# vismaychuriwala/Fast-Image-Editing-with-Generative-Models

Measured on AMD Instinct MI355X. Metric: PIE-Bench images/sec @1024^2 SSD-1B fp16 4-step, higher is better.
Workload: dtype f16

## Files before the change

fast-image-editing-with-generative-models_amd/csrc/fie_internal.h:

```cpp
#pragma once
#include <hip/hip_runtime.h>
#include <stdint.h>
#include <stdio.h>
#include <string.h>
#include <map>
#include <string>
#include <tuple>
#include <utility>
#include <vector>
#include "../../include/fie.h"

typedef _Float16 half_t;
typedef _Float16 f16x8 __attribute__((ext_vector_type(8)));
typedef _Float16 f16x4 __attribute__((ext_vector_type(4)));
typedef _Float16 f16x2 __attribute__((ext_vector_type(2)));
typedef float f32x4 __attribute__((ext_vector_type(4)));
typedef short s16x4 __attribute__((ext_vector_type(4)));
typedef unsigned u32x4 __attribute__((ext_vector_type(4)));

struct fie_launch_rec {
    const void* fn;
    dim3 grid, block;
    unsigned lds;
    std::vector<unsigned char> blob;
// ... 19 lines not shown
};

struct fie_ctx {
    int device;
    hipStream_t stream;
    int num_cus;
    int force_tile = 0;
    int gemm_probe = 0;
    int epi_prefetch = 1;
    unsigned* gemm_stamps = nullptr;
    float* gn_target = nullptr;
    int64_t gn_target_rows = 0;
    int gn_target_groups = 0;
    int attn_variant = 0;
    int gn_onepass = 1;
    unsigned* err_flag = nullptr;
    void* sk_ws = nullptr;
    int64_t sk_bytes = 0;
    int splitk_mode = 1;
    int autotune = 0;
    std::map<fie_tune_key, int> tuned;
    int tune_exclude[16] = {0};
    void* tune_buf = nullptr;
    void* tune_flush = nullptr;
    size_t tune_bytes = 0;
    int n_overrides = 0;
    fie_tile_override overrides[32];
    char last_kernel[128] = "";
    fie_program* recording = nullptr;
    std::vector<std::string>* oplog = nullptr;
// ... 94 lines not shown
```

fast-image-editing-with-generative-models_amd/csrc/graphs.cpp:

```cpp
#include <string>
#include <vector>

#include "fie_internal.h"

namespace {

struct Arena {
    struct Blk { int64_t off, size; bool used; };
    std::vector<Blk> blks;
    int64_t high = 0;
    explicit Arena(int64_t cap) { blks.push_back({0, cap, false}); }
    int64_t take(int64_t bytes) {
        bytes = fie_roundup(bytes > 0 ? bytes : 1, 256);
        for (size_t i = 0; i < blks.size(); ++i) {
            if (blks[i].used || blks[i].size < bytes) continue;
            const int64_t off = blks[i].off, rest = blks[i].size - bytes;
            blks[i].size = bytes;
            blks[i].used = true;
            if (rest > 0) blks.insert(blks.begin() + i + 1, Blk{off + bytes, rest, false});
            if (off + bytes > high) high = off + bytes;
            return off;
        }
        return -1;
    }
// ... 27 lines not shown
    int rc = FIE_OK;
    bool plan_fused = true;
    char* cache = nullptr;
    int64_t cache_cap = 0, cache_cur = 0;
    bool cache_fill = false, cache_count = false;
    bool cached() const { return cache != nullptr || cache_count; }
    T cache_slot(int64_t rows, int c) {
        T t;
        t.rows = rows; t.c = c;
        const int64_t bytes = fie_roundup(rows * c * 2, 256);
        if (!cache_count && cache_cur + bytes > cache_cap && rc == FIE_OK) { fie_set_error("%s: step cache too small (fie_unet_step_cache_bytes)", who); rc = FIE_EINVAL; }
        t.ext = cache_count || !ok() ? reinterpret_cast<void*>(1) : static_cast<void*>(cache + cache_cur);
        cache_cur += bytes;
        return t;
    }
    Walk(fie_ctx* c, const char* w, const char* pre, void* ws, int64_t cap) : ctx(c), who(w), prefix(pre ? pre : ""), base(static_cast<char*>(ws)), arena(cap) {}
    bool plan() const { return ctx == nullptr; }
    bool ok() const { return rc == FIE_OK; }
    void run(int r) { if (rc == FIE_OK && r != FIE_OK) rc = r; }

    T alloc(int64_t rows, int c) {
        T t;
        t.rows = rows; t.c = c;
        t.off = arena.take(rows * c * 2);
        if (t.off < 0 && rc == FIE_OK) { fie_set_error("%s: workspace too small", who); rc = FIE_EINVAL; t.off = 0; }
        return t;
    }
    int64_t scratch(int64_t bytes) {
        int64_t off = arena.take(bytes);
        if (off < 0 && rc == FIE_OK) { fie_set_error("%s: workspace too small", who); rc = FIE_EINVAL; off = 0; }
        return off;
// ... 685 lines not shown
```

fast-image-editing-with-generative-models_amd/csrc/norm.hip:

```cpp
#include "fie_internal.h"

namespace {

constexpr int GN_THREADS = 256;
constexpr int GN_MAX_CHUNKS = 1024;

template <typename T>
struct GnArgsT {
    const T* X1; int C1;
    const T* X2; int C2;
    T* Y;
    int C, G, cg;
    int64_t rows;
    int rows_per_chunk, nchunks;
    int ncol;
    int rpp;
    const T* gamma; const T* beta;
    float eps; int silu;
    float* partial;
    float* stats;
    float o8_inv;
    int pg;
};

using GnArgs = GnArgsT<half_t>;

__device__ __forceinline__ int gn_pack4_f8(const float* o, float inv) {
    auto q = [&](float x) { return fie_sat448(x * inv); };
    int pk = __builtin_amdgcn_cvt_pk_fp8_f32(q(o[0]), q(o[1]), 0, false);
    return __builtin_amdgcn_cvt_pk_fp8_f32(q(o[2]), q(o[3]), pk, true);
}

template <typename T>
__device__ __forceinline__ void gn_load(const GnArgsT<T>& p, int64_t row_global, int c0, float (&x)[8]) {
    if (c0 < p.C1) fie_load8(p.X1 + row_global * p.C1 + c0, x);
    else fie_load8(p.X2 + row_global * p.C2 + (c0 - p.C1), x);
}

template <typename T>
__global__ __launch_bounds__(GN_THREADS) void gn_partial_kernel(GnArgsT<T> p) {
    __shared__ float red[GN_THREADS * 16];
    const int tid = threadIdx.x;
    const int col = tid % p.ncol, rsub = tid / p.ncol;
    const int b = blockIdx.y;
    const int c0 = (blockIdx.z * p.ncol + col) * 8;
    const bool active = rsub < p.rpp && c0 < p.C;
    float s[8], ss[8];
#pragma unroll
    for (int j = 0; j < 8; ++j) s[j] = ss[j] = 0.f;
    if (active) {
        const int64_t r_begin = (int64_t)blockIdx.x * p.rows_per_chunk;
// ... 16 lines not shown
    __syncthreads();
    const int cbase = blockIdx.z * p.ncol * 8;
    const int cend = min(cbase + p.ncol * 8, p.C);
    const int g_first = cbase / p.cg, g_last = (cend - 1) / p.cg;
    for (int g = g_first + tid; g <= g_last; g += GN_THREADS) {
        float a = 0.f, q = 0.f;
        const int ch_lo = max(g * p.cg, cbase), ch_hi = min((g + 1) * p.cg, cend);
        for (int ch = ch_lo; ch < ch_hi; ++ch) {
            const int lc = (ch - cbase) >> 3, j = (ch - cbase) & 7;
            for (int rs = 0; rs < p.rpp; ++rs) {
                a += red[(rs * p.ncol + lc) * 16 + j];
                q += red[(rs * p.ncol + lc) * 16 + 8 + j];
            }
        }
        float* dst = p.partial + (((int64_t)b * p.nchunks + blockIdx.x) * p.G + g) * 2;
        dst[0] = a;
        dst[1] = q;
    }
}

template <typename T>
__global__ __launch_bounds__(256) void gn_finalize_kernel(GnArgsT<T> p, int B) {
    const int lane = threadIdx.x & 63;
    const int i = blockIdx.x * 4 + (threadIdx.x >> 6);
    if (i >= B * p.G) return;
    const int b = i / p.G, g = i - b * p.G;
    double a = 0.0, q = 0.0;
    for (int c = lane; c < p.nchunks; c += 64) {
        const float2 v = *reinterpret_cast<const float2*>(p.partial + (((int64_t)b * p.nchunks + c) * p.G + g) * 2);
        a += (double)v.x;
        q += (double)v.y;
    }
#pragma unroll
    for (int o = 32; o > 0; o >>= 1) {
        a += __shfl_xor(a, o);
        q += __shfl_xor(q, o);
    }
    if (lane == 0) {
        const double n = (double)p.rows * p.cg;
        const double mean = a / n;
        double var = q / n - mean * mean;
        if (var < 0.0) var = 0.0;
        p.stats[i * 2] = (float)mean;
        p.stats[i * 2 + 1] = (float)(1.0 / sqrt(var + (double)p.eps));
    }
}

template <typename T>
__global__ __launch_bounds__(256) void gn_finalize_wide_kernel(GnArgsT<T> p, int B) {
    __shared__ double red[8];
    const int tid = threadIdx.x, lane = tid & 63, wave = tid >> 6;
    const int i = blockIdx.x;
    const int b = i / p.G, g = i - b * p.G;
    double a0 = 0.0, q0 = 0.0, a1 = 0.0, q1 = 0.0, a2 = 0.0, q2 = 0.0, a3 = 0.0, q3 = 0.0;
    if (p.pg > p.G) {
        const int upg = p.pg / p.G;
        const float2* src = reinterpret_cast<const float2*>(p.partial) + (int64_t)b * p.nchunks * p.pg + g * upg;
        const int total = p.nchunks * upg;
        for (int i = tid; i < total; i += 256) {
            const int c = i / upg, u = i - c * upg;
// ... 39 lines not shown
    const int tid = threadIdx.x, g = tid % p.G, sub = tid / p.G, nsub = 256 / p.G;
    const int b = blockIdx.y, c0 = blockIdx.x * per, c1 = min(c0 + per, ngran);
    const float2* src = reinterpret_cast<const float2*>(granules) + (int64_t)b * ngran * p.G + g;
    double a0 = 0.0, q0 = 0.0, a1 = 0.0, q1 = 0.0;
    int c = c0 + sub;
    for (; c + nsub < c1; c += 2 * nsub) {
        const float2 v0 = src[(int64_t)c * p.G], v1 = src[(int64_t)(c + nsub) * p.G];
        a0 += (double)v0.x; q0 += (double)v0.y; a1 += (double)v1.x; q1 += (double)v1.y;
    }
    if (c < c1) { const float2 v = src[(int64_t)c * p.G]; a0 += (double)v.x; q0 += (double)v.y; }
    red[tid][0] = a0 + a1; red[tid][1] = q0 + q1;
    __syncthreads();
    if (sub == 0) {
        double a = 0.0, q = 0.0;
        for (int s = 0; s < nsub; ++s) { a += red[s * p.G + g][0]; q += red[s * p.G + g][1]; }
        *reinterpret_cast<float2*>(p.partial + (((int64_t)b * gridDim.x + blockIdx.x) * p.G + g) * 2) = make_float2((float)a, (float)q);
    }
}

template <typename T>
__global__ __launch_bounds__(GN_THREADS) void gn_apply_kernel(GnArgsT<T> p) {
    const int tid = threadIdx.x;
    const int col = tid % p.ncol, rsub = tid / p.ncol;
    const int b = blockIdx.y;
    const int c0 = (blockIdx.z * p.ncol + col) * 8;
    if (!(rsub < p.rpp && c0 < p.C)) return;
    float sc[8], sh[8];
    float gm[8], bt[8];
    fie_load8(p.gamma + c0, gm);
    fie_load8(p.beta + c0, bt);
#pragma unroll
    for (int j = 0; j < 8; ++j) {
// ... 239 lines not shown
                fie_store8(Y + row * ldy + ch * 8, o);
            }
        }
    }
}

template <typename T, bool O8, typename... Args>
void ln_launch(fie_ctx* ctx, int64_t rows, int C, Args... args) {
    const dim3 grid((unsigned)((rows + 3) / 4)), block(256);
    if (C <= 1024) fie_launch(ctx, (ln_kernel<T, O8, 2>), grid, block, 0, args...);
    else if (C <= 1536) fie_launch(ctx, (ln_kernel<T, O8, 3>), grid, block, 0, args...);
    else fie_launch(ctx, (ln_kernel<T, O8, LN_MAXV>), grid, block, 0, args...);
}

template <typename T>
int gn_plan(GnArgsT<T>& p, int C, int G, int64_t rows, int B, int* csplit) {
    const int nc8 = C / 8;
    int split = (nc8 + GN_THREADS - 1) / GN_THREADS;
    while (split <= nc8 && (nc8 % split != 0 || ((nc8 / split) * 8) % (C / G) != 0)) ++split;
    if (split > nc8) return -1;
    p.ncol = nc8 / split;
    p.rpp = GN_THREADS / p.ncol;
    *csplit = split;
    int64_t want = 2048 / (B > 0 ? B : 1);
    if (want < 1) want = 1;
    if (want > GN_MAX_CHUNKS) want = GN_MAX_CHUNKS;
    int64_t rpc = fie_roundup((rows + want - 1) / want, p.rpp);
    int64_t nch = (rows + rpc - 1) / rpc;
    p.rows_per_chunk = (int)rpc;
    p.nchunks = (int)nch;
    return 0;
}

template <typename T>
int groupnorm_t(const char* who, fie_ctx* ctx, const void* X1, int C1, const void* X2, int C2, void* Y, int B, int64_t rows_per_image,
                int groups, const void* gamma, const void* beta, float eps, int silu, void* workspace, float o8_inv = 0.f) {
    FIE_REQUIRE(ctx && X1 && Y && gamma && beta && workspace, "%s: NULL argument", who);
    FIE_REQUIRE(C1 > 0 && C1 % 8 == 0 && C2 >= 0 && C2 % 8 == 0 && (C2 == 0 || X2), "%s: C1=%d C2=%d invalid", who, C1, C2);
    const int C = C1 + C2;
    FIE_REQUIRE(B > 0 && rows_per_image > 0 && groups > 0 && C % groups == 0, "%s: bad shape C=%d G=%d", who, C, groups);
    GnArgsT<T> p = {};
    p.X1 = (const T*)X1; p.C1 = C1; p.X2 = (const T*)X2; p.C2 = C2; p.Y = (T*)Y;
    p.C = C; p.G = groups; p.cg = C / groups; p.rows = rows_per_image;
    p.gamma = (const T*)gamma; p.beta = (const T*)beta; p.eps = eps; p.silu = silu;
    p.o8_inv = o8_inv;
    int csplit = 1;
    FIE_REQUIRE(gn_plan(p, C, groups, rows_per_image, B, &csplit) == 0, "%s: cannot split C=%d (groups=%d) into aligned column blocks", who, C, groups);
    if (ctx->gn_onepass && gn_onepass(ctx, p, B)) {
        FIE_LAUNCH_CHECK();
        return FIE_OK;
    }
    p.partial = (float*)workspace;
    p.stats = p.partial + (int64_t)B * GN_MAX_CHUNKS * groups * 2;
    const dim3 grid((unsigned)p.nchunks, (unsigned)B, (unsigned)csplit);
    FIE_DESC(ctx, "groupnorm partial B=%d rows=%lld C=%d G=%d bytes=%.0f", B, (long long)rows_per_image, C, groups, 1.0 * B * rows_per_image * C * sizeof(T));
    fie_launch(ctx, gn_partial_kernel<T>, grid, dim3(GN_THREADS), 0, p);
    FIE_DESC(ctx, "groupnorm finalize B=%d rows=%lld C=%d G=%d bytes=0", B, (long long)rows_per_image, C, groups);
    fie_launch(ctx, gn_finalize_kernel<T>, dim3((B * groups + 3) / 4), dim3(256), 0, p, B);
    FIE_DESC(ctx, "groupnorm apply B=%d rows=%lld C=%d G=%d bytes=%.0f", B, (long long)rows_per_image, C, groups, 2.0 * B * rows_per_image * C * sizeof(T));
    fie_launch(ctx, gn_apply_kernel<T>, grid, dim3(GN_THREADS), 0, p);
    FIE_LAUNCH_CHECK();
    return FIE_OK;
}

template <typename T>
int layernorm_t(const char* who, fie_ctx* ctx, const void* X, int64_t ldx, void* Y, int64_t ldy, int64_t rows, int C, const void* gamma,
                const void* beta, float eps) {
    FIE_REQUIRE(ctx && X && Y && gamma && beta, "%s: NULL argument", who);
    FIE_REQUIRE(rows > 0 && C > 0 && C % 8 == 0 && C <= 64 * 8 * LN_MAXV, "%s: C=%d unsupported", who, C);
    FIE_REQUIRE(ldx % 8 == 0 && ldy % 8 == 0 && ldx >= C && ldy >= C, "%s: bad strides", who);
    FIE_DESC(ctx, "layernorm rows=%lld C=%d bytes=%.0f", (long long)rows, C, 2.0 * rows * C * sizeof(T));
    ln_launch<T, false>(ctx, rows, C, (const T*)X, ldx, (T*)Y, ldy, rows, C, (const T*)gamma, (const T*)beta, eps, 1.f);
    FIE_LAUNCH_CHECK();
// ... 4 lines not shown

template <typename T>
int groupnorm_stats_t(const char* who, fie_ctx* ctx, const void* X, int C, void* Y, int B, int64_t rows_per_image, int groups, const void* gamma,
                      const void* beta, float eps, int silu, const void* partial, void* workspace, int partial_groups, float o8_inv = 0.f) {
    FIE_REQUIRE(ctx && X && Y && gamma && beta && partial && workspace, "%s: NULL argument", who);
    FIE_REQUIRE(C > 0 && C % 8 == 0 && B > 0 && groups > 0 && C % groups == 0 && rows_per_image > 0 && rows_per_image % 32 == 0,
                "%s: bad shape C=%d G=%d rows=%lld", who, C, groups, (long long)rows_per_image);
    GnArgsT<T> p = {};
    p.X1 = (const T*)X; p.C1 = C; p.X2 = nullptr; p.C2 = 0; p.Y = (T*)Y;
    p.C = C; p.G = groups; p.cg = C / groups; p.rows = rows_per_image;
    p.gamma = (const T*)gamma; p.beta = (const T*)beta; p.eps = eps; p.silu = silu;
    p.o8_inv = o8_inv;
    int csplit = 1;
    FIE_REQUIRE(gn_plan(p, C, groups, rows_per_image, B, &csplit) == 0, "%s: cannot split C=%d (groups=%d) into aligned column blocks", who, C, groups);
    const dim3 grid((unsigned)p.nchunks, (unsigned)B, (unsigned)csplit);
    p.stats = (float*)workspace + (int64_t)B * GN_MAX_CHUNKS * groups * 2;
    GnArgsT<T> f = p;
    f.partial = const_cast<float*>((const float*)partial);
    f.nchunks = (int)(rows_per_image / 32);
    FIE_REQUIRE(partial_groups == 0 || partial_groups == groups || (partial_groups > groups && partial_groups % groups == 0 && partial_groups * 4 == C),
                "%s: partial_groups=%d must be 0, the group count, or C / 4 quads divisible into the %d groups", who, partial_groups, groups);
    f.pg = partial_groups;
    const int ngran = (int)(rows_per_image / 32);
    if (ngran >= 4096 && groups <= 256 && 256 % groups == 0 && partial_groups <= groups) {
        const int nb = 256, per = (ngran + nb - 1) / nb;
        GnArgsT<T> g2 = p;
        g2.partial = (float*)workspace;
        g2.nchunks = nb;
        FIE_DESC(ctx, "groupnorm gather-granules B=%d rows=%lld C=%d G=%d bytes=%.0f", B, (long long)rows_per_image, C, groups, 8.0 * B * ngran * groups);
        fie_launch(ctx, gn_gather_granules_kernel<T>, dim3(nb, B), dim3(256), 0, g2, (const float*)partial, ngran, per);
        FIE_DESC(ctx, "groupnorm finalize B=%d rows=%lld C=%d G=%d bytes=0", B, (long long)rows_per_image, C, groups);
        fie_launch(ctx, gn_finalize_kernel<T>, dim3((B * groups + 3) / 4), dim3(256), 0, g2, B);
    } else {
        FIE_DESC(ctx, "groupnorm finalize-from-epilogue B=%d rows=%lld C=%d G=%d bytes=0", B, (long long)rows_per_image, C, groups);
        fie_launch(ctx, gn_finalize_wide_kernel<T>, dim3(B * groups), dim3(256), 0, f, B);
    }
    FIE_DESC(ctx, "groupnorm apply B=%d rows=%lld C=%d G=%d bytes=%.0f", B, (long long)rows_per_image, C, groups, 2.0 * B * rows_per_image * C * sizeof(T));
    fie_launch(ctx, gn_apply_kernel<T>, grid, dim3(GN_THREADS), 0, p);
    FIE_LAUNCH_CHECK();
    return FIE_OK;
}

namespace {
template <typename T>
__global__ __launch_bounds__(256) void gn_coef_kernel(GnArgsT<T> p, float* coef) {
    const int b = blockIdx.y, c = blockIdx.x * 256 + threadIdx.x;
    if (c >= p.C) return;
// ... 6 lines not shown
}

extern "C" {

int fie_groupnorm_coef_f16(fie_ctx* ctx, int C, int B, int64_t rows_per_image, int groups, const void* gamma, const void* beta, float eps, const void* partial,
                           void* workspace, int partial_groups, float* coef) {
    const char* who = "fie_groupnorm_coef_f16";
    FIE_REQUIRE(ctx && gamma && beta && partial && workspace && coef, "%s: NULL argument", who);
    FIE_REQUIRE(C > 0 && C % 8 == 0 && B > 0 && groups > 0 && C % groups == 0 && rows_per_image > 0 && rows_per_image % 32 == 0,
                "%s: bad shape C=%d G=%d rows=%lld", who, C, groups, (long long)rows_per_image);
    FIE_REQUIRE(partial_groups == 0 || partial_groups == groups || (partial_groups > groups && partial_groups % groups == 0 && partial_groups * 4 == C),
                "%s: partial_groups=%d must be 0, the group count, or C / 4 quads divisible into the %d groups", who, partial_groups, groups);
    GnArgs p = {};
    p.C1 = C; p.C = C; p.G = groups; p.cg = C / groups; p.rows = rows_per_image;
    p.gamma = (const half_t*)gamma; p.beta = (const half_t*)beta; p.eps = eps;
    p.stats = (float*)workspace + (int64_t)B * GN_MAX_CHUNKS * groups * 2;
    const int ngran = (int)(rows_per_image / 32);
    if (ngran >= 4096 && groups <= 256 && 256 % groups == 0 && partial_groups <= groups) {
        const int nb = 256, per = (ngran + nb - 1) / nb;
        GnArgs g2 = p;
        g2.partial = (float*)workspace;
        g2.nchunks = nb;
        FIE_DESC(ctx, "groupnorm gather-granules B=%d rows=%lld C=%d G=%d bytes=%.0f", B, (long long)rows_per_image, C, groups, 8.0 * B * ngran * groups);
        fie_launch(ctx, gn_gather_granules_kernel<half_t>, dim3(nb, B), dim3(256), 0, g2, (const float*)partial, ngran, per);
        FIE_DESC(ctx, "groupnorm finalize B=%d rows=%lld C=%d G=%d bytes=0", B, (long long)rows_per_image, C, groups);
        fie_launch(ctx, gn_finalize_kernel<half_t>, dim3((B * groups + 3) / 4), dim3(256), 0, g2, B);
    } else {
        GnArgs f = p;
        f.partial = const_cast<float*>((const float*)partial);
        f.nchunks = ngran;
        f.pg = partial_groups;
        FIE_DESC(ctx, "groupnorm finalize-from-epilogue B=%d rows=%lld C=%d G=%d bytes=0", B, (long long)rows_per_image, C, groups);
        fie_launch(ctx, gn_finalize_wide_kernel<half_t>, dim3(B * groups), dim3(256), 0, f, B);
    }
    FIE_DESC(ctx, "groupnorm coefficients B=%d rows=%lld C=%d G=%d bytes=0", B, (long long)rows_per_image, C, groups);
    fie_launch(ctx, gn_coef_kernel<half_t>, dim3((C + 255) / 256, B), dim3(256), 0, p, coef);
    FIE_LAUNCH_CHECK();
    return FIE_OK;
}

int64_t fie_gn_stats_bytes(int B, int64_t rows_per_image, int groups) { return (int64_t)B * (rows_per_image / 32) * groups * 2 * (int64_t)sizeof(float); }

int fie_groupnorm_stats_nhwc_f16(fie_ctx* ctx, const void* X, int C, void* Y, int B, int64_t rows_per_image, int groups, const void* gamma,
// ... 5 lines not shown
int fie_groupnorm_nhwc_f16_o8(fie_ctx* ctx, const void* X1, int C1, const void* X2, int C2, void* Y8, int B, int64_t rows_per_image, int groups,
                              const void* gamma, const void* beta, float eps, int silu, void* workspace, float inv_scale) {
    FIE_REQUIRE(inv_scale > 0.f, "fie_groupnorm_nhwc_f16_o8: inv_scale must be positive");
    return groupnorm_t<half_t>("fie_groupnorm_nhwc_f16_o8", ctx, X1, C1, X2, C2, Y8, B, rows_per_image, groups, gamma, beta, eps, silu, workspace, inv_scale);
}

int fie_groupnorm_stats_nhwc_f16_o8(fie_ctx* ctx, const void* X, int C, void* Y8, int B, int64_t rows_per_image, int groups, const void* gamma,
                                    const void* beta, float eps, int silu, const void* partial, void* workspace, int partial_groups, float inv_scale) {
    FIE_REQUIRE(inv_scale > 0.f, "fie_groupnorm_stats_nhwc_f16_o8: inv_scale must be positive");
    return groupnorm_stats_t<half_t>("fie_groupnorm_stats_nhwc_f16_o8", ctx, X, C, Y8, B, rows_per_image, groups, gamma, beta, eps, silu, partial, workspace,
                                     partial_groups, inv_scale);
}

int64_t fie_groupnorm_workspace_bytes(int B, int64_t rows_per_image, int groups) {
    (void)rows_per_image;
    return ((int64_t)B * GN_MAX_CHUNKS * groups * 2 + (int64_t)B * groups * 2) * (int64_t)sizeof(float);
}

int fie_groupnorm_nhwc_f16(fie_ctx* ctx, const void* X1, int C1, const void* X2, int C2, void* Y, int B,
                           int64_t rows_per_image, int groups, const void* gamma, const void* beta, float eps,
                           int silu, void* workspace) {
    return groupnorm_t<half_t>("fie_groupnorm_nhwc_f16", ctx, X1, C1, X2, C2, Y, B, rows_per_image, groups, gamma, beta, eps, silu, workspace);
}

int fie_groupnorm_nhwc_f32(fie_ctx* ctx, const void* X1, int C1, const void* X2, int C2, void* Y, int B,
                           int64_t rows_per_image, int groups, const void* gamma, const void* beta, float eps,
                           int silu, void* workspace) {
    return groupnorm_t<float>("fie_groupnorm_nhwc_f32", ctx, X1, C1, X2, C2, Y, B, rows_per_image, groups, gamma, beta, eps, silu, workspace);
}

int fie_layernorm_f16(fie_ctx* ctx, const void* X, int64_t ldx, void* Y, int64_t ldy, int64_t rows, int C,
// ... 8 lines not shown

int fie_layernorm_f16_o8(fie_ctx* ctx, const void* X, int64_t ldx, void* Y8, int64_t ldy8, int64_t rows, int C, const void* gamma, const void* beta,
                         float eps, float inv_scale) {
    const char* who = "fie_layernorm_f16_o8";
    FIE_REQUIRE(ctx && X && Y8 && gamma && beta, "%s: NULL argument", who);
    FIE_REQUIRE(rows > 0 && C > 0 && C % 8 == 0 && C <= 64 * 8 * LN_MAXV && inv_scale > 0.f, "%s: C=%d unsupported", who, C);
    FIE_REQUIRE(ldx % 8 == 0 && ldy8 % 8 == 0 && ldx >= C && ldy8 >= C, "%s: bad strides", who);
    FIE_DESC(ctx, "layernorm->e4m3 rows=%lld C=%d bytes=%.0f", (long long)rows, C, 3.0 * rows * C);
    ln_launch<half_t, true>(ctx, rows, C, (const half_t*)X, ldx, (half_t*)Y8, ldy8, rows, C, (const half_t*)gamma, (const half_t*)beta, eps, inv_scale);
    FIE_LAUNCH_CHECK();
    return FIE_OK;
}

}

extern "C" int fie_debug_gn_onepass(fie_ctx* ctx, int enable) {
    FIE_REQUIRE(ctx != nullptr, "fie_debug_gn_onepass: NULL ctx");
    ctx->gn_onepass = enable;
    return FIE_OK;
}
```

fast-image-editing-with-generative-models_amd/hip.py:

```python
import ctypes
import os
import subprocess

import torch

_CSRC = os.path.join(os.path.dirname(os.path.abspath(__file__)), "csrc")
LIB_PATH = os.environ.get("FIE_LIB_PATH") or os.path.join(_CSRC, "libfie_hip.so")

ACT_NONE, ACT_SILU, ACT_GELU, ACT_QUICK_GELU, ACT_GEGLU = 0, 1, 2, 3, 4

_c = ctypes
_P, _I, _L, _F = _c.c_void_p, _c.c_int, _c.c_int64, _c.c_float

SIGNATURES = {
    "fie_version": [],
    "fie_ctx_create": [_I, _P, _c.POINTER(_P)],
    "fie_ctx_set_stream": [_P, _P],
    "fie_ctx_error_flag": [_P, _P],
    "fie_ctx_destroy": [_P],
    "fie_weights_register": [_P, _c.c_char_p, _P, _L, _L],
    "fie_weights_clear": [_P],
    "fie_vae_decode_workspace_bytes": [_P, _I, _I],
    "fie_vae_decode_f16": [_P, _P, _P, _P, _P, _L],
    "fie_vae_encode_workspace_bytes": [_P],
# ... 83 lines not shown
    "fie_metrics_pairs_u8": [_P, _P, _P, _P, _I, _I, _I, _P, _P, _L],
    "fie_clip_mask_rgb_u8": [_P, _P, _P, _I, _I, _I, _I, _I, _P, _P, _P],
    "fie_clip_patches_u8_f16": [_P, _P, _I, _I, _I, _I, _I, _I, _I, _P, _P, _P],
    "fie_clip_patches_u8_f32": [_P, _P, _I, _I, _I, _I, _I, _I, _I, _P, _P, _P],
    "fie_vit_embed_f16": [_P, _P, _P, _P, _I, _I, _I, _P],
    "fie_vit_embed_f32": [_P, _P, _P, _P, _I, _I, _I, _P],
    "fie_clip_score_f16": [_P, _P, _L, _P, _L, _I, _I, _P],
    "fie_clip_score_f32": [_P, _P, _L, _P, _L, _I, _I, _P],
    "fie_dino_patches_u8_f16": [_P, _P, _I, _I, _I, _I, _I, _P, _P, _I, _P, _P, _I, _I, _P, _P, _P, _P],
    "fie_dino_patches_u8_f32": [_P, _P, _I, _I, _I, _I, _I, _P, _P, _I, _P, _P, _I, _I, _P, _P, _P, _P],
    "fie_selfsim_workspace_bytes": [_I, _I],
    "fie_selfsim_mse_f16": [_P, _P, _P, _L, _I, _I, _I, _P, _P],
    "fie_selfsim_mse_f32": [_P, _P, _P, _L, _I, _I, _I, _P, _P],
    "fie_debug_force_tile": [_P, _I],
    "fie_debug_attn_variant": [_P, _I],
    "fie_debug_gn_onepass": [_P, _I],
    "fie_debug_tile_override": [_P, _c.c_char_p],
    "fie_debug_last_gemm_kernel": [_P],
    "fie_prefetch": [_P, _P, _L, _P, _I],
    "fie_conv3x3_plus_nhwc_f16": [_P, _P, _I, _I, _I, _I, _P, _L, _P, _L, _I, _P, _P, _L, _F, _I, _P, _L, _I, _P, _L, _I],
    "fie_conv_up2x_nhwc_f16": [_P, _P, _I, _I, _I, _I, _P, _L, _I, _P, _L, _I, _P, _P, _L, _F, _I],
    "fie_gn_stats_target": [_P, _P, _L, _I],
    "fie_gn_stats_bytes": [_I, _L, _I],
    "fie_groupnorm_stats_nhwc_f16": [_P, _P, _I, _P, _I, _L, _I, _P, _P, _F, _I, _P, _P, _I],
    "fie_gemm_autotune": [_P, _I],
    "fie_gemm_autotune_report": [_P, ctypes.c_char_p, _I],
    "fie_gemm_autotune_load": [_P, ctypes.c_char_p],
    "fie_debug_tune_exclude": [_P, ctypes.c_char_p],
    "fie_debug_gemm_probe": [_P, _I],
    "fie_debug_epilogue_prefetch": [_P, _I],
# ... 98 lines not shown
        return lib().fie_program_launches(self.h)

    def run(self):
        self.ctx.sync_stream()
        _chk(lib().fie_program_run(self.ctx.h, self.h))
        return self.outputs

    def register(self, name):
        assert name in GRAPH_NAMES, name
        _chk(lib().fie_graph_register(self.ctx.h, name.encode(), self.h))

    def close(self):
        if self.h:
            lib().fie_program_destroy(self.ctx.h, self.h)
            self.h = _P()


class W8:

    def __init__(self, q, scale):
        self.q, self.scale = q, scale

    def stride(self, d):
        return self.q.stride(d)

    def dequant(self):
        return self.q.view(torch.float8_e4m3fn).float() * self.scale[:, None]


class Context:
# ... 80 lines not shown
        key = (self._stream, self.ws_tag)
        if key == self._sk_bound:
            return
        ws = self._sk_ws.get(key)
        if ws is None:
            ws = self._sk_ws[key] = torch.zeros(self.splitk_bytes, device=self.device, dtype=torch.uint8)
        _chk(lib().fie_splitk_workspace(self.h, ws.data_ptr(), ws.numel()))
        self._sk_bound = key

    def capture_stream(self):
        if self._cap_stream is None:
            self._cap_stream = torch.cuda.Stream(device=self.device)
        with torch.cuda.stream(self._cap_stream):
            self.sync_stream()
            self._bind_splitk()
        torch.cuda.synchronize(self.device)
        return self._cap_stream

    def splitk_counters_clear(self):
        torch.cuda.synchronize(self.device)
        live = list(self._sk_ws.values()) + [w for w in (r() for r in self._prog_ws) if w is not None]
        return all(int(ws[:16384].view(torch.int32).abs().max()) == 0 for ws in live)

    def record(self):
        import contextlib

        @contextlib.contextmanager
        def cm():
            prog = Program(self)
            self.sync_stream()
# ... 302 lines not shown
                                    0, None, 0, 1.0, ACT_NONE, batch, heads, tq * q.stride(0), d, tk * k.stride(0), d,
                                    heads * tq * tk, tq * tk))
            _chk(lib().fie_softmax_rows_f32(self.h, _p(s_), batch * heads * tq, tk, tk, float(scale), int(causal), tq))
            _chk(lib().fie_gemm_f32(self.h, _p(s_), tk, tk, None, 0, _p(v), v.stride(0), 1, _p(out), out.stride(0), tq, d, tk, None,
                                    None, 0, 0, None, 0, 1.0, ACT_NONE, batch, heads, heads * tq * tk, tq * tk, tk * v.stride(0), d,
                                    tq * out.stride(0), d))
            return out
        if out_f8:
            _chk(lib().fie_attention_f16_o8(self.h, _p(q), q.stride(0), _p(k), k.stride(0), _p(v), v.stride(0), _p(out), out.stride(0), batch, heads, tq, tk,
                                            head_dim, float(scale), int(causal), float(out_inv_scale)))
            return out
        _chk(lib().fie_attention_f16(self.h, _p(q), q.stride(0), _p(k), k.stride(0), _p(v), v.stride(0), _p(out),
                                     out.stride(0), batch, heads, tq, tk, head_dim, float(scale), int(causal)))
        return out

    def groupnorm(self, x1, gamma, beta, groups, eps, silu, x2=None, out=None, out_f8=False, out_inv_scale=1.0):
        self.sync_stream()
        b, rows, c1 = x1.shape[0], x1[0].numel() // x1.shape[-1], x1.shape[-1]
        c2 = x2.shape[-1] if x2 is not None else 0
        assert x1.is_contiguous() and (x2 is None or x2.is_contiguous())
        if out is None:
            out = self._alloc(x1.shape[:-1] + (c1 + c2,), torch.uint8 if out_f8 else None)
        need = lib().fie_groupnorm_workspace_bytes(b, rows, groups)
        key = (self._stream, self.ws_tag)
        ws = self._gn_ws.get(key)
        if ws is None or ws.numel() < need:
            ws = self._gn_ws[key] = torch.empty(need, device=self.device, dtype=torch.uint8)
        if self._keep is not None:
            self._keep.append(ws)
        tag = getattr(x1, "_gn_tag", None)
        if (tag is not None and x2 is None and tag[1:5] == (groups, c1, rows, b) and tag[5] == self._gn_gen and tag[6] == key):
            if out_f8:
                _chk(lib().fie_groupnorm_stats_nhwc_f16_o8(self.h, _p(x1), c1, _p(out), b, rows, groups, _p(gamma), _p(beta), float(eps), int(silu),
                                                           _p(tag[0]), _p(ws), tag[7], float(out_inv_scale)))
                return out
            _chk(lib().fie_groupnorm_stats_nhwc_f16(self.h, _p(x1), c1, _p(out), b, rows, groups, _p(gamma), _p(beta), float(eps), int(silu),
                                                    _p(tag[0]), _p(ws), tag[7]))
            return out
        if out_f8:
            _chk(lib().fie_groupnorm_nhwc_f16_o8(self.h, _p(x1), c1, _p(x2), c2, _p(out), b, rows, groups, _p(gamma), _p(beta), float(eps), int(silu), _p(ws),
                                                 float(out_inv_scale)))
            return out
        _chk((lib().fie_groupnorm_nhwc_f32 if self.f32 else lib().fie_groupnorm_nhwc_f16)(self.h, _p(x1), c1, _p(x2), c2, _p(out), b, rows, groups, _p(gamma),
                                          _p(beta), float(eps), int(silu), _p(ws)))
        return out

    def conv3x3_gn_ok(self, x, cout, out_groups):
        b, h, w, cin = x.shape
        return bool(self.gn_fuse_conv and not self.f32 and getattr(x, "_gn_tag", None) is not None and out_groups
                    and lib().fie_conv3x3_gn_ok(self.h, b, h, w, cin, cout, out_groups))

    def groupnorm_coef(self, x, gamma, beta, groups, eps):
        self.sync_stream()
        b, rows, c = x.shape[0], x[0].numel() // x.shape[-1], x.shape[-1]
        tag = getattr(x, "_gn_tag", None)
        key = (self._stream, self.ws_tag)
        if not (tag is not None and tag[1:5] == (groups, c, rows, b) and tag[5] == self._gn_gen and tag[6] == key):
            return None
        need = lib().fie_groupnorm_workspace_bytes(b, rows, groups)
        ws = self._gn_ws.get(key)
        if ws is None or ws.numel() < need:
            ws = self._gn_ws[key] = torch.empty(need, device=self.device, dtype=torch.uint8)
        if self._keep is not None:
            self._keep.append(ws)
        coef = self._alloc((b, c, 2), torch.float32)
        _chk(lib().fie_groupnorm_coef_f16(self.h, c, b, rows, groups, _p(gamma), _p(beta), float(eps), _p(tag[0]), _p(ws), tag[7], _p(coef)))
        return coef

    def conv3x3_gn(self, x, coef, silu, wp, cout, bias=None, residual=None, gn_groups=None):
        self.sync_stream()
        self._bind_splitk()
        b, h, w, cin = x.shape
        assert x.is_contiguous() and coef.dtype == torch.float32 and coef.shape == (b, cin, 2)
        out = self._alloc((b, h, w, cout))
        tag = self._gn_stats_arm(b * h * w, cout, h * w, gn_groups)
        assert tag is not None, "the fused GroupNorm -> conv needs the output's sums armed (conv3x3_gn_ok)"
        _chk(lib().fie_conv3x3_gn_nhwc_f16(self.h, _p(x), b, h, w, cin, _p(coef), int(bool(silu)), _p(wp), wp.stride(0), _p(out), out.stride(2), cout, _p(bias),
# ... 313 lines not shown
```

include/fie.h:

```cpp
#ifndef FIE_H_
#define FIE_H_

#include <stdint.h>

#ifdef __cplusplus
extern "C" {
#endif

#define FIE_OK 0
#define FIE_EINVAL (-1)
#define FIE_EHIP (-2)
#define FIE_ENODEV (-3)

#define FIE_DEVERR_TIME_EMBED_BARRIER 1u

#define FIE_ACT_NONE 0
#define FIE_ACT_SILU 1
#define FIE_ACT_GELU 2
#define FIE_ACT_QUICK_GELU 3
#define FIE_ACT_GEGLU 4

typedef struct fie_ctx fie_ctx;

int fie_version(void);
// ... 211 lines not shown
int fie_debug_splitk(fie_ctx* ctx, int mode);
int fie_gemm_autotune(fie_ctx* ctx, int on);
int fie_gemm_autotune_report(fie_ctx* ctx, char* buf, int cap);
int fie_gemm_autotune_load(fie_ctx* ctx, const char* text);
int fie_debug_tune_exclude(fie_ctx* ctx, const char* codes);
int fie_debug_gemm_probe(fie_ctx* ctx, int mode);
int fie_debug_epilogue_prefetch(fie_ctx* ctx, int on);
int fie_debug_gemm_stamps(fie_ctx* ctx, void* buf);
const char* fie_debug_last_gemm_kernel(fie_ctx* ctx);
int fie_debug_oplog(fie_ctx* ctx, int on);
int fie_debug_oplog_mark(fie_ctx* ctx, const char* text);
int64_t fie_debug_oplog_read(fie_ctx* ctx, char* buf, int64_t cap);
int fie_debug_tune_candidates(fie_ctx* ctx, int on);
int64_t fie_debug_tune_candidates_read(fie_ctx* ctx, char* buf, int64_t cap);
int fie_debug_attn_variant(fie_ctx* ctx, int variant);
int fie_debug_gn_onepass(fie_ctx* ctx, int enable);

int fie_canny_rgb_u8(const uint8_t* rgb, int H, int W, int low, int high, uint8_t* edges_rgb);

int64_t fie_canny_workspace_bytes(int H, int W);
int fie_canny_rgb_device_u8(fie_ctx* ctx, const uint8_t* rgb, int H, int W, int low, int high, void* workspace,
                            uint8_t* edges_rgb, int* iterations);
int fie_canny_rgb_device_begin_u8(fie_ctx* ctx, const uint8_t* rgb, int H, int W, int low, int high, int rounds, void* workspace, uint8_t* edges_rgb,
                                  int* host_flags);
int fie_canny_rgb_device_finish_u8(fie_ctx* ctx, int H, int W, void* workspace, uint8_t* edges_rgb, int* host_flags, int* iterations);

int fie_resize_rgb_u8(fie_ctx* ctx, const uint8_t* src, int H, int W, uint8_t* dst, int OH, int OW, const int* kx,
                      const int* bx, int ksx, const int* ky, const int* by, int ksy, uint8_t* tmp);

int fie_resize_l_u8(fie_ctx* ctx, const uint8_t* src, int H, int W, uint8_t* dst, int OH, int OW, const int* kx,
// ... 51 lines not shown
```

Before: 15.42.

## Fuse GroupNorm finalize into partial kernel via last-block atomic ticket

```diff
diff --git a/fast-image-editing-with-generative-models_amd/csrc/fie_internal.h b/fast-image-editing-with-generative-models_amd/csrc/fie_internal.h
--- a/fast-image-editing-with-generative-models_amd/csrc/fie_internal.h
+++ b/fast-image-editing-with-generative-models_amd/csrc/fie_internal.h
@@ -57,6 +57,8 @@
     int gn_target_groups = 0;
     int attn_variant = 0;
     int gn_onepass = 1;
+    int gn_ticket = 1;
+    unsigned* gn_tickets = nullptr;
     unsigned* err_flag = nullptr;
     void* sk_ws = nullptr;
     int64_t sk_bytes = 0;
diff --git a/fast-image-editing-with-generative-models_amd/csrc/gn_plan.h b/fast-image-editing-with-generative-models_amd/csrc/gn_plan.h
--- /dev/null
+++ b/fast-image-editing-with-generative-models_amd/csrc/gn_plan.h
@@ -0,0 +1,30 @@
+#pragma once
+#include <stdint.h>
+
+constexpr int GN_THREADS = 256;
+constexpr int GN_MAX_CHUNKS = 1024;
+constexpr int GN_TICKET_WORDS = 256;
+
+constexpr int64_t gn_ws_partial_offset() { return (int64_t)GN_TICKET_WORDS * (int64_t)sizeof(unsigned); }
+inline int64_t gn_ws_stats_offset(int B, int G) { return gn_ws_partial_offset() + (int64_t)B * GN_MAX_CHUNKS * G * 2 * (int64_t)sizeof(float); }
+inline int64_t gn_ws_bytes(int B, int G) { return gn_ws_stats_offset(B, G) + (int64_t)B * G * 2 * (int64_t)sizeof(float); }
+
+template <typename P>
+int gn_plan(P& p, int C, int G, int64_t rows, int B, int* csplit) {
+    const int nc8 = C / 8;
+    int split = (nc8 + GN_THREADS - 1) / GN_THREADS;
+    while (split <= nc8 && (nc8 % split != 0 || ((nc8 / split) * 8) % (C / G) != 0)) ++split;
+    if (split > nc8) return -1;
+    p.ncol = nc8 / split;
+    p.rpp = GN_THREADS / p.ncol;
+    *csplit = split;
+    int64_t want = 2048 / ((int64_t)(B > 0 ? B : 1) * split);
+    if (want < 1) want = 1;
+    if (want > GN_MAX_CHUNKS) want = GN_MAX_CHUNKS;
+    int64_t rpc = (rows + want - 1) / want;
+    rpc = (rpc + p.rpp - 1) / p.rpp * p.rpp;
+    int64_t nch = (rows + rpc - 1) / rpc;
+    p.rows_per_chunk = (int)rpc;
+    p.nchunks = (int)nch;
+    return 0;
+}
diff --git a/fast-image-editing-with-generative-models_amd/csrc/graphs.cpp b/fast-image-editing-with-generative-models_amd/csrc/graphs.cpp
--- a/fast-image-editing-with-generative-models_amd/csrc/graphs.cpp
+++ b/fast-image-editing-with-generative-models_amd/csrc/graphs.cpp
@@ -65,7 +65,22 @@
         cache_cur += bytes;
         return t;
     }
-    Walk(fie_ctx* c, const char* w, const char* pre, void* ws, int64_t cap) : ctx(c), who(w), prefix(pre ? pre : ""), base(static_cast<char*>(ws)), arena(cap) {}
+    static constexpr int64_t kGnTicketBytes = 1024;
+    int gn_ticket_saved = 1;
+    Walk(fie_ctx* c, const char* w, const char* pre, void* ws, int64_t cap) : ctx(c), who(w), prefix(pre ? pre : ""), base(static_cast<char*>(ws)), arena(cap) {
+        const int64_t tk = scratch(kGnTicketBytes);
+        if (!ctx) return;
+        gn_ticket_saved = ctx->gn_ticket;
+        if (!ok() || ctx->recording || !ctx->gn_ticket || hipMemsetAsync(base + tk, 0, kGnTicketBytes, ctx->stream) != hipSuccess) ctx->gn_ticket = 0;
+        else ctx->gn_tickets = reinterpret_cast<unsigned*>(base + tk);
+    }
+    ~Walk() {
+        if (!ctx) return;
+        ctx->gn_tickets = nullptr;
+        ctx->gn_ticket = gn_ticket_saved;
+    }
+    Walk(const Walk&) = delete;
+    Walk& operator=(const Walk&) = delete;
     bool plan() const { return ctx == nullptr; }
     bool ok() const { return rc == FIE_OK; }
     void run(int r) { if (rc == FIE_OK && r != FIE_OK) rc = r; }
diff --git a/fast-image-editing-with-generative-models_amd/csrc/norm.hip b/fast-image-editing-with-generative-models_amd/csrc/norm.hip
--- a/fast-image-editing-with-generative-models_amd/csrc/norm.hip
+++ b/fast-image-editing-with-generative-models_amd/csrc/norm.hip
@@ -1,9 +1,7 @@
 #include "fie_internal.h"
+#include "gn_plan.h"
 
 namespace {
-
-constexpr int GN_THREADS = 256;
-constexpr int GN_MAX_CHUNKS = 1024;
 
 template <typename T>
 struct GnArgsT {
@@ -20,6 +18,7 @@
     float* partial;
     float* stats;
     float o8_inv;
+    unsigned* tickets;
     int pg;
 };
 
@@ -35,6 +34,61 @@
 __device__ __forceinline__ void gn_load(const GnArgsT<T>& p, int64_t row_global, int c0, float (&x)[8]) {
     if (c0 < p.C1) fie_load8(p.X1 + row_global * p.C1 + c0, x);
     else fie_load8(p.X2 + row_global * p.C2 + (c0 - p.C1), x);
+}
+
+__device__ __forceinline__ void gn_store_partial(float* dst, float a, float q, bool through) {
+    if (through) {
+        const unsigned long long u = (unsigned long long)__float_as_uint(a) | ((unsigned long long)__float_as_uint(q) << 32);
+        __hip_atomic_store(reinterpret_cast<unsigned long long*>(dst), u, __ATOMIC_RELAXED, __HIP_MEMORY_SCOPE_AGENT);
+    } else {
+        *reinterpret_cast<float2*>(dst) = make_float2(a, q);
+    }
+}
+
+__device__ __forceinline__ bool gn_last_ticket(unsigned* counter, unsigned n, volatile unsigned* flag) {
+    asm volatile("s_waitcnt vmcnt(0)" ::: "memory");
+    __syncthreads();
+    if (threadIdx.x == 0) *flag = __hip_atomic_fetch_add(counter, 1u, __ATOMIC_RELAXED, __HIP_MEMORY_SCOPE_AGENT);
+    __syncthreads();
+    if (*flag % n != n - 1) return false;
+    if (threadIdx.x == 0) {
+        (void)__hip_atomic_fetch_sub(counter, n, __ATOMIC_RELAXED, __HIP_MEMORY_SCOPE_AGENT);
+        __builtin_amdgcn_fence(__ATOMIC_ACQUIRE, "agent");
+    }
+    asm volatile("s_waitcnt vmcnt(0)" ::: "memory");
+    __syncthreads();
+    return true;
+}
+
+template <bool THROUGH, typename T>
+__device__ __forceinline__ void gn_finalize_group(const GnArgsT<T>& p, int b, int g, int lane) {
+    double a = 0.0, q = 0.0;
+    for (int c = lane; c < p.nchunks; c += 64) {
+        const float* src = p.partial + (((int64_t)b * p.nchunks + c) * p.G + g) * 2;
+        float2 v;
+        if constexpr (THROUGH) {
+            const unsigned long long u = __hip_atomic_load(reinterpret_cast<const unsigned long long*>(src), __ATOMIC_RELAXED, __HIP_MEMORY_SCOPE_AGENT);
+            v = make_float2(__uint_as_float((unsigned)u), __uint_as_float((unsigned)(u >> 32)));
+        } else {
+            v = *reinterpret_cast<const float2*>(src);
+        }
+        a += (double)v.x;
+        q += (double)v.y;
+    }
+#pragma unroll
+    for (int o = 32; o > 0; o >>= 1) {
+        a += __shfl_xor(a, o);
+        q += __shfl_xor(q, o);
+    }
+    if (lane == 0) {
+        const int i = b * p.G + g;
+        const double n = (double)p.rows * p.cg;
+        const double mean = a / n;
+        double var = q / n - mean * mean;
+        if (var < 0.0) var = 0.0;
+        p.stats[i * 2] = (float)mean;
+        p.stats[i * 2 + 1] = (float)(1.0 / sqrt(var + (double)p.eps));
+    }
 }
 
 template <typename T>
@@ -81,36 +135,18 @@
             }
         }
         float* dst = p.partial + (((int64_t)b * p.nchunks + blockIdx.x) * p.G + g) * 2;
-        dst[0] = a;
-        dst[1] = q;
-    }
+        gn_store_partial(dst, a, q, p.tickets != nullptr);
+    }
+    if (!p.tickets) return;
+    if (!gn_last_ticket(p.tickets + b * gridDim.z + blockIdx.z, gridDim.x, reinterpret_cast<volatile unsigned*>(red))) return;
+    for (int g = g_first + (tid >> 6); g <= g_last; g += GN_THREADS / 64) gn_finalize_group<true>(p, b, g, tid & 63);
 }
 
 template <typename T>
 __global__ __launch_bounds__(256) void gn_finalize_kernel(GnArgsT<T> p, int B) {
-    const int lane = threadIdx.x & 63;
     const int i = blockIdx.x * 4 + (threadIdx.x >> 6);
     if (i >= B * p.G) return;
-    const int b = i / p.G, g = i - b * p.G;
-    double a = 0.0, q = 0.0;
-    for (int c = lane; c < p.nchunks; c += 64) {
-        const float2 v = *reinterpret_cast<const float2*>(p.partial + (((int64_t)b * p.nchunks + c) * p.G + g) * 2);
-        a += (double)v.x;
-        q += (double)v.y;
-    }
-#pragma unroll
-    for (int o = 32; o > 0; o >>= 1) {
-        a += __shfl_xor(a, o);
-        q += __shfl_xor(q, o);
-    }
-    if (lane == 0) {
-        const double n = (double)p.rows * p.cg;
-        const double mean = a / n;
-        double var = q / n - mean * mean;
-        if (var < 0.0) var = 0.0;
-        p.stats[i * 2] = (float)mean;
-        p.stats[i * 2 + 1] = (float)(1.0 / sqrt(var + (double)p.eps));
-    }
+    gn_finalize_group<false>(p, i / p.G, i % p.G, threadIdx.x & 63);
 }
 
 template <typename T>
@@ -180,8 +216,11 @@
     if (sub == 0) {
         double a = 0.0, q = 0.0;
         for (int s = 0; s < nsub; ++s) { a += red[s * p.G + g][0]; q += red[s * p.G + g][1]; }
-        *reinterpret_cast<float2*>(p.partial + (((int64_t)b * gridDim.x + blockIdx.x) * p.G + g) * 2) = make_float2((float)a, (float)q);
-    }
+        gn_store_partial(p.partial + (((int64_t)b * gridDim.x + blockIdx.x) * p.G + g) * 2, (float)a, (float)q, p.tickets != nullptr);
+    }
+    if (!p.tickets) return;
+    if (!gn_last_ticket(p.tickets + b, gridDim.x, reinterpret_cast<volatile unsigned*>(&red[0][0]))) return;
+    for (int gg = tid >> 6; gg < p.G; gg += 4) gn_finalize_group<true>(p, b, gg, tid & 63);
 }
 
 template <typename T>
@@ -451,22 +490,10 @@
 }
 
 template <typename T>
-int gn_plan(GnArgsT<T>& p, int C, int G, int64_t rows, int B, int* csplit) {
-    const int nc8 = C / 8;
-    int split = (nc8 + GN_THREADS - 1) / GN_THREADS;
-    while (split <= nc8 && (nc8 % split != 0 || ((nc8 / split) * 8) % (C / G) != 0)) ++split;
-    if (split > nc8) return -1;
-    p.ncol = nc8 / split;
-    p.rpp = GN_THREADS / p.ncol;
-    *csplit = split;
-    int64_t want = 2048 / (B > 0 ? B : 1);
-    if (want < 1) want = 1;
-    if (want > GN_MAX_CHUNKS) want = GN_MAX_CHUNKS;
-    int64_t rpc = fie_roundup((rows + want - 1) / want, p.rpp);
-    int64_t nch = (rows + rpc - 1) / rpc;
-    p.rows_per_chunk = (int)rpc;
-    p.nchunks = (int)nch;
-    return 0;
+void gn_workspace(const fie_ctx* ctx, GnArgsT<T>& p, void* workspace, int B, int64_t counters) {
+    p.partial = reinterpret_cast<float*>(static_cast<char*>(workspace) + gn_ws_partial_offset());
+    p.stats = reinterpret_cast<float*>(static_cast<char*>(workspace) + gn_ws_stats_offset(B, p.G));
+    p.tickets = sizeof(T) == 2 && ctx->gn_ticket && counters <= GN_TICKET_WORDS ? (ctx->gn_tickets ? ctx->gn_tickets : static_cast<unsigned*>(workspace)) : nullptr;
 }
 
 template <typename T>
@@ -487,13 +514,14 @@
         FIE_LAUNCH_CHECK();
         return FIE_OK;
     }
-    p.partial = (float*)workspace;
-    p.stats = p.partial + (int64_t)B * GN_MAX_CHUNKS * groups * 2;
+    gn_workspace(ctx, p, workspace, B, (int64_t)B * csplit);
     const dim3 grid((unsigned)p.nchunks, (unsigned)B, (unsigned)csplit);
     FIE_DESC(ctx, "groupnorm partial B=%d rows=%lld C=%d G=%d bytes=%.0f", B, (long long)rows_per_image, C, groups, 1.0 * B * rows_per_image * C * sizeof(T));
     fie_launch(ctx, gn_partial_kernel<T>, grid, dim3(GN_THREADS), 0, p);
-    FIE_DESC(ctx, "groupnorm finalize B=%d rows=%lld C=%d G=%d bytes=0", B, (long long)rows_per_image, C, groups);
-    fie_launch(ctx, gn_finalize_kernel<T>, dim3((B * groups + 3) / 4), dim3(256), 0, p, B);
+    if (!p.tickets) {
+        FIE_DESC(ctx, "groupnorm finalize B=%d rows=%lld C=%d G=%d bytes=0", B, (long long)rows_per_image, C, groups);
+        fie_launch(ctx, gn_finalize_kernel<T>, dim3((B * groups + 3) / 4), dim3(256), 0, p, B);
+    }
     FIE_DESC(ctx, "groupnorm apply B=%d rows=%lld C=%d G=%d bytes=%.0f", B, (long long)rows_per_image, C, groups, 2.0 * B * rows_per_image * C * sizeof(T));
     fie_launch(ctx, gn_apply_kernel<T>, grid, dim3(GN_THREADS), 0, p);
     FIE_LAUNCH_CHECK();
@@ -528,9 +556,10 @@
     int csplit = 1;
     FIE_REQUIRE(gn_plan(p, C, groups, rows_per_image, B, &csplit) == 0, "%s: cannot split C=%d (groups=%d) into aligned column blocks", who, C, groups);
     const dim3 grid((unsigned)p.nchunks, (unsigned)B, (unsigned)csplit);
-    p.stats = (float*)workspace + (int64_t)B * GN_MAX_CHUNKS * groups * 2;
+    gn_workspace(ctx, p, workspace, B, B);
     GnArgsT<T> f = p;
     f.partial = const_cast<float*>((const float*)partial);
+    f.tickets = nullptr;
     f.nchunks = (int)(rows_per_image / 32);
     FIE_REQUIRE(partial_groups == 0 || partial_groups == groups || (partial_groups > groups && partial_groups % groups == 0 && partial_groups * 4 == C),
                 "%s: partial_groups=%d must be 0, the group count, or C / 4 quads divisible into the %d groups", who, partial_groups, groups);
@@ -539,12 +568,13 @@
     if (ngran >= 4096 && groups <= 256 && 256 % groups == 0 && partial_groups <= groups) {
         const int nb = 256, per = (ngran + nb - 1) / nb;
         GnArgsT<T> g2 = p;
-        g2.partial = (float*)workspace;
         g2.nchunks = nb;
         FIE_DESC(ctx, "groupnorm gather-granules B=%d rows=%lld C=%d G=%d bytes=%.0f", B, (long long)rows_per_image, C, groups, 8.0 * B * ngran * groups);
         fie_launch(ctx, gn_gather_granules_kernel<T>, dim3(nb, B), dim3(256), 0, g2, (const float*)partial, ngran, per);
-        FIE_DESC(ctx, "groupnorm finalize B=%d rows=%lld C=%d G=%d bytes=0", B, (long long)rows_per_image, C, groups);
-        fie_launch(ctx, gn_finalize_kernel<T>, dim3((B * groups + 3) / 4), dim3(256), 0, g2, B);
+        if (!g2.tickets) {
+            FIE_DESC(ctx, "groupnorm finalize B=%d rows=%lld C=%d G=%d bytes=0", B, (long long)rows_per_image, C, groups);
+            fie_launch(ctx, gn_finalize_kernel<T>, dim3((B * groups + 3) / 4), dim3(256), 0, g2, B);
+        }
     } else {
         FIE_DESC(ctx, "groupnorm finalize-from-epilogue B=%d rows=%lld C=%d G=%d bytes=0", B, (long long)rows_per_image, C, groups);
         fie_launch(ctx, gn_finalize_wide_kernel<T>, dim3(B * groups), dim3(256), 0, f, B);
@@ -581,19 +611,21 @@
     GnArgs p = {};
     p.C1 = C; p.C = C; p.G = groups; p.cg = C / groups; p.rows = rows_per_image;
     p.gamma = (const half_t*)gamma; p.beta = (const half_t*)beta; p.eps = eps;
-    p.stats = (float*)workspace + (int64_t)B * GN_MAX_CHUNKS * groups * 2;
+    gn_workspace(ctx, p, workspace, B, B);
     const int ngran = (int)(rows_per_image / 32);
     if (ngran >= 4096 && groups <= 256 && 256 % groups == 0 && partial_groups <= groups) {
         const int nb = 256, per = (ngran + nb - 1) / nb;
         GnArgs g2 = p;
-        g2.partial = (float*)workspace;
         g2.nchunks = nb;
         FIE_DESC(ctx, "groupnorm gather-granules B=%d rows=%lld C=%d G=%d bytes=%.0f", B, (long long)rows_per_image, C, groups, 8.0 * B * ngran * groups);
         fie_launch(ctx, gn_gather_granules_kernel<half_t>, dim3(nb, B), dim3(256), 0, g2, (const float*)partial, ngran, per);
-        FIE_DESC(ctx, "groupnorm finalize B=%d rows=%lld C=%d G=%d bytes=0", B, (long long)rows_per_image, C, groups);
-        fie_launch(ctx, gn_finalize_kernel<half_t>, dim3((B * groups + 3) / 4), dim3(256), 0, g2, B);
+        if (!g2.tickets) {
+            FIE_DESC(ctx, "groupnorm finalize B=%d rows=%lld C=%d G=%d bytes=0", B, (long long)rows_per_image, C, groups);
+            fie_launch(ctx, gn_finalize_kernel<half_t>, dim3((B * groups + 3) / 4), dim3(256), 0, g2, B);
+        }
     } else {
         GnArgs f = p;
+        f.tickets = nullptr;
         f.partial = const_cast<float*>((const float*)partial);
         f.nchunks = ngran;
         f.pg = partial_groups;
@@ -629,7 +661,7 @@
 
 int64_t fie_groupnorm_workspace_bytes(int B, int64_t rows_per_image, int groups) {
     (void)rows_per_image;
-    return ((int64_t)B * GN_MAX_CHUNKS * groups * 2 + (int64_t)B * groups * 2) * (int64_t)sizeof(float);
+    return gn_ws_bytes(B, groups);
 }
 
 int fie_groupnorm_nhwc_f16(fie_ctx* ctx, const void* X1, int C1, const void* X2, int C2, void* Y, int B,
@@ -668,6 +700,12 @@
 
 }
 
+extern "C" int fie_debug_gn_ticket(fie_ctx* ctx, int enable) {
+    FIE_REQUIRE(ctx != nullptr, "fie_debug_gn_ticket: NULL ctx");
+    ctx->gn_ticket = enable ? 1 : 0;
+    return FIE_OK;
+}
+
 extern "C" int fie_debug_gn_onepass(fie_ctx* ctx, int enable) {
     FIE_REQUIRE(ctx != nullptr, "fie_debug_gn_onepass: NULL ctx");
     ctx->gn_onepass = enable;
diff --git a/fast-image-editing-with-generative-models_amd/hip.py b/fast-image-editing-with-generative-models_amd/hip.py
--- a/fast-image-editing-with-generative-models_amd/hip.py
+++ b/fast-image-editing-with-generative-models_amd/hip.py
@@ -121,6 +121,7 @@
     "fie_selfsim_mse_f32": [_P, _P, _P, _L, _I, _I, _I, _P, _P],
     "fie_debug_force_tile": [_P, _I],
     "fie_debug_attn_variant": [_P, _I],
+    "fie_debug_gn_ticket": [_P, _I],
     "fie_debug_gn_onepass": [_P, _I],
     "fie_debug_tile_override": [_P, _c.c_char_p],
     "fie_debug_last_gemm_kernel": [_P],
@@ -249,6 +250,9 @@
         if self.h:
             lib().fie_program_destroy(self.ctx.h, self.h)
             self.h = _P()
+
+
+GN_TICKET_BYTES = 1024
 
 
 class W8:
@@ -359,6 +363,8 @@
         with torch.cuda.stream(self._cap_stream):
             self.sync_stream()
             self._bind_splitk()
+            if self._gn_ws:
+                self._gn_workspace(max(w.numel() for w in self._gn_ws.values()))
         torch.cuda.synchronize(self.device)
         return self._cap_stream
 
@@ -691,6 +697,14 @@
                                      out.stride(0), batch, heads, tq, tk, head_dim, float(scale), int(causal)))
         return out
 
+    def _gn_workspace(self, need):
+        key = (self._stream, self.ws_tag)
+        ws = self._gn_ws.get(key)
+        if ws is None or ws.numel() < need:
+            ws = self._gn_ws[key] = torch.empty(need, device=self.device, dtype=torch.uint8)
+            ws[:GN_TICKET_BYTES].zero_()
+        return ws
+
     def groupnorm(self, x1, gamma, beta, groups, eps, silu, x2=None, out=None, out_f8=False, out_inv_scale=1.0):
         self.sync_stream()
         b, rows, c1 = x1.shape[0], x1[0].numel() // x1.shape[-1], x1.shape[-1]
@@ -699,13 +713,11 @@
         if out is None:
             out = self._alloc(x1.shape[:-1] + (c1 + c2,), torch.uint8 if out_f8 else None)
         need = lib().fie_groupnorm_workspace_bytes(b, rows, groups)
-        key = (self._stream, self.ws_tag)
-        ws = self._gn_ws.get(key)
-        if ws is None or ws.numel() < need:
-            ws = self._gn_ws[key] = torch.empty(need, device=self.device, dtype=torch.uint8)
+        ws = self._gn_workspace(need)
         if self._keep is not None:
             self._keep.append(ws)
         tag = getattr(x1, "_gn_tag", None)
+        key = (self._stream, self.ws_tag)
         if (tag is not None and x2 is None and tag[1:5] == (groups, c1, rows, b) and tag[5] == self._gn_gen and tag[6] == key):
             if out_f8:
                 _chk(lib().fie_groupnorm_stats_nhwc_f16_o8(self.h, _p(x1), c1, _p(out), b, rows, groups, _p(gamma), _p(beta), float(eps), int(silu),
@@ -735,9 +747,7 @@
         if not (tag is not None and tag[1:5] == (groups, c, rows, b) and tag[5] == self._gn_gen and tag[6] == key):
             return None
         need = lib().fie_groupnorm_workspace_bytes(b, rows, groups)
-        ws = self._gn_ws.get(key)
-        if ws is None or ws.numel() < need:
-            ws = self._gn_ws[key] = torch.empty(need, device=self.device, dtype=torch.uint8)
+        ws = self._gn_workspace(need)
         if self._keep is not None:
             self._keep.append(ws)
         coef = self._alloc((b, c, 2), torch.float32)
diff --git a/include/fie.h b/include/fie.h
--- a/include/fie.h
+++ b/include/fie.h
@@ -249,6 +249,7 @@
 int fie_debug_tune_candidates(fie_ctx* ctx, int on);
 int64_t fie_debug_tune_candidates_read(fie_ctx* ctx, char* buf, int64_t cap);
 int fie_debug_attn_variant(fie_ctx* ctx, int variant);
+int fie_debug_gn_ticket(fie_ctx* ctx, int enable);
 int fie_debug_gn_onepass(fie_ctx* ctx, int enable);
 
 int fie_canny_rgb_u8(const uint8_t* rgb, int H, int W, int low, int high, uint8_t* edges_rgb);
```

After: 15.02. -2.6%, worse.
